# hasindu2008/sigfish

Hardware: AMD Instinct MI355X
Metric: reads/s (sDTW alignment stage: nCoV-2019 R9 DNA, -q 250, both strands) (higher is better)
Workload: dtype f32

## Files before the change

### sigfish_amd/csrc/sdtw_kernels.hpp

```cpp
#pragma once

#include <hip/hip_runtime.h>
#include <stddef.h>
#include <stdint.h>

#include "row_rules.hpp"

namespace sfa {

constexpr int kRefPad = 128;
#ifndef SFA_STEPS_PER_LOAD
#define SFA_STEPS_PER_LOAD 4
#endif
#ifndef SFA_FILL_WAVES
#define SFA_FILL_WAVES 6
#endif
#ifndef SFA_FILL32_WAVES
#define SFA_FILL32_WAVES 4
#endif
#ifndef SFA_LCK_WAVES
#define SFA_LCK_WAVES 4
#endif
#ifndef SFA_TRACE_WAVES
#define SFA_TRACE_WAVES 4
// ... 1169 lines not shown
template <int MAXR, bool STD, bool LCK = false>
__global__ void __launch_bounds__(256, MAXR <= 16 ? SFA_TRACE_WAVES : 1) sdtw_trace_kernel(const DpArgs a, int32_t *out_st) {
    const int task = __builtin_amdgcn_readfirstlane(blockIdx.x * 4 + (threadIdx.x >> 6));
    if (task >= a.n_tasks) return;
    int ci = 0;
    while (ci + 1 < a.n_cls && task >= a.cls[ci + 1].task_base) ++ci;
    const ClassDesc cd = a.cls[ci];
    const int tl = task - cd.task_base;
    __shared__ float lds_f[4 * kXchWordsPerWave];
    __shared__ int lds_i[4 * kXchWordsPerWave];
#define SFA_SHAPE(RR, LL)                                                                    \
    case (RR) * 256 + (LL):                                                                  \
        if constexpr (MAXR >= (RR)) trace_body<RR, LL, STD, LCK>(a, cd, tl, out_st, lds_f, lds_i); \
        break;
    switch (cd.R * 256 + cd.lanes) {
        SFA_SHAPE(32, 64) SFA_SHAPE(32, 32) SFA_SHAPE(32, 16)
        SFA_SHAPE(16, 64) SFA_SHAPE(16, 32) SFA_SHAPE(16, 16)
        SFA_SHAPE(8, 64) SFA_SHAPE(8, 32) SFA_SHAPE(8, 16)
        SFA_SHAPE(4, 64) SFA_SHAPE(4, 32)
        default:
            trace_body<4, 16, STD, LCK>(a, cd, tl, out_st, lds_f, lds_i);
            break;
    }
#undef SFA_SHAPE
}

template <int R, int L, bool STD, bool LCK>
__device__ __forceinline__ void fused_trace_task(const DpArgs &a, const ClassDesc cd, const int quad_local, float *lds_f, int *lds_i, float *lds_x) {
    const int quad = cd.quad_base + quad_local;
    const int lane = threadIdx.x & 63;
    const int g = lane & (L - 1);
    const int slot = lane / L;
    int seen;
    const bool arrived = bounded_wait_ge(a.quad_done + quad, a.n_chunks, a.spin_limit, &seen, true);
    __builtin_amdgcn_fence(__ATOMIC_ACQUIRE, "agent");
    __builtin_amdgcn_wave_barrier();
    if (!arrived) {
        if (lane == 0) report_device_error(a.err, kErrQuadWait, quad, seen);
        return;
    }
    const int qlen = __builtin_amdgcn_readfirstlane(a.quad_qlen[quad]);
    const int lq = (qlen - 1) / R;
    const int read = a.order[quad * 4 + slot];
    const bool owner = (g == lq) && read >= 0;
    ResultRow r = no_row();
    Winner w;
    w.job = -1;
    w.ws = -1;
    w.best = 0.0f;
    w.chunk = 0;
    if (owner && !a.bad[read]) {
        float best = INFINITY, second = INFINITY;
        int end = -1, job = -1, chunk = 0;
        for (int ch = 0; ch < a.n_chunks; ++ch) {
            const int64_t o = (static_cast<int64_t>(quad) * a.n_chunks + ch) * 4 + slot;
            const float b = a.p_best[o], s2 = a.p_second[o];
            const float hi = fmaxf(best, b);
            const float lo2 = fminf(second, s2);
            const bool take = !(b > best);
            second = fminf(hi, lo2);
            if (take) {
                best = b;
                end = a.p_end[o];
                job = a.p_job[o];
                chunk = ch;
            }
        }
        r.valid = 1;
        r.score = best;
        r.score2 = second;
        if (job >= 0) {
            r.rid = a.job_contig[job];
            r.strand = a.job_strand[job];
            r.mapq = mapq_from_scores(best, second);
            w.job = job;
            w.ws = end;
            w.best = best;
            w.chunk = chunk;
        }
    }
    const int src = (lane & ~(L - 1)) + lq;
    w.job = __shfl(w.job, src);
    w.ws = __shfl(w.ws, src);
    w.best = __shfl(w.best, src);
    w.chunk = __shfl(w.chunk, src);
    int res_st, res_end;
    trace_core<R, L, STD, LCK, (R == 32)>(a, cd, quad_local, w, lds_f, lds_i, res_st, res_end, lds_x);
    if (owner) {
        if (r.rid >= 0) {
            const int rl = a.ref_len[r.rid], off = a.ref_st_offset[r.rid];
            r.pos_st = ((r.strand == '+') ? res_st : rl - res_end) + off;
            r.pos_end = ((r.strand == '+') ? res_end : rl - res_st) + off;
            if (a.span_hist && res_st >= 0 && res_end >= res_st) {
                const int64_t ql = a.q_off[read + 1] - a.q_off[read];
                if (ql > 0) {
                    const int64_t b = (static_cast<int64_t>(res_end - res_st + 1) * 16) / ql;
                    atomicAdd(a.span_hist + (b < kSpanBuckets - 1 ? static_cast<int>(b) : kSpanBuckets - 1), 1u);
                }
            }
        }
        a.out[read] = r;
    }
}

template <int MAXR, bool STD, bool LCK>
__device__ __attribute__((noinline)) void fused_trace_dispatch(const DpArgs *pa, const int quad, float *lds_f, int *lds_i, float *lds_x) {
    const DpArgs &a = *pa;
    int ci = 0;
    while (ci + 1 < a.n_cls && quad >= a.cls[ci + 1].quad_base) ++ci;
    const ClassDesc cd = a.cls[ci];
    const int ql = quad - cd.quad_base;
#define SFA_TSHAPE(RR, LL)                                                               \
    case (RR) * 256 + (LL):                                                              \
        if constexpr (MAXR >= (RR)) fused_trace_task<RR, LL, STD, LCK>(a, cd, ql, lds_f, lds_i, lds_x); \
        break;
    switch (cd.R * 256 + cd.lanes) {
        SFA_TSHAPE(32, 64) SFA_TSHAPE(32, 32) SFA_TSHAPE(32, 16)
        SFA_TSHAPE(16, 64) SFA_TSHAPE(16, 32) SFA_TSHAPE(16, 16)
        SFA_TSHAPE(8, 64) SFA_TSHAPE(8, 32) SFA_TSHAPE(8, 16)
        SFA_TSHAPE(4, 64) SFA_TSHAPE(4, 32) SFA_TSHAPE(4, 16)
        default:
            break;
    }
#undef SFA_TSHAPE
}

struct SecArgs {
    const int32_t *slot_of_read;
    const int32_t *p_top5;
    const uint8_t *bad;
    const int64_t *q_off;
    int32_t max_query;
    int32_t n_reads, n_chunks;
    int32_t *s_job;
    int32_t *s_end;
// ... 29 lines not shown
    if (w >= static_cast<int64_t>(n_quads_total) * per_quad) return;
    const int quad = static_cast<int>(w / per_quad), rest = static_cast<int>(w - static_cast<int64_t>(quad) * per_quad);
    const int job = rest / (a.n_seg - 1), seg = rest - job * (a.n_seg - 1);
    int ci = 0;
    while (ci + 1 < a.n_cls && quad >= a.cls[ci + 1].quad_base) ++ci;
    const int qlen = a.quad_qlen[quad];
    const SegRange next = segment_range(a.job_len[job], qlen, a.n_seg, a.warm_windows, seg + 1);
    if (next.empty) return;
    const int lane = threadIdx.x & 63;
    const float *out = a.verify + verify_slot(a, quad, job, seg, 1) + lane, *in = a.verify + verify_slot(a, quad, job, seg + 1, 0) + lane;
    bool same = true;
    for (int p = 0; p <= a.cls[ci].R; ++p) same = same && (__float_as_uint(out[p * 64]) == __float_as_uint(in[p * 64]));
    if (!__all(same) && lane == 0) a.seg_fail[quad] = 1;
}

__global__ void __launch_bounds__(256) sdtw_screen_kernel(const float *queries, const int64_t *q_off, const int n, uint8_t *bad,
                                                          unsigned *count) {
    const int i = blockIdx.x * 4 + (threadIdx.x >> 6);
    if (i >= n) return;
    const int lane = threadIdx.x & 63;
    const int64_t b = q_off[i], e = q_off[i + 1];
    bool nf = false;
    for (int64_t j = b + lane; j < e; j += 64) {
        const unsigned u = __float_as_uint(queries[j]);
        nf = nf || ((u & 0x7f800000u) == 0x7f800000u);
    }
    const bool any = __any(nf);
    if (lane == 0) {
        bad[i] = any ? 1 : 0;
        if (any) atomicAdd(count, 1u);
    }
}

struct ChunkWin {
    int end, job, chunk;
};
__global__ void __launch_bounds__(256) sdtw_finalize_kernel(const FinalizeArgs a) {
    const int i = blockIdx.x * blockDim.x + threadIdx.x;
    if (i >= a.n_reads) return;
    const int sl = a.slot_of_read[i];
    const int64_t qlen = a.q_off[i + 1] - a.q_off[i];
    const bool strips = a.max_query > 0 && qlen > a.max_query;
    if (strips && a.mode != 1) return;
    if (a.mode == 3) {
        if (sl < 0) a.out[i] = no_row();
        return;
    }
    if (a.mode == 2) {
        if (sl < 0) return;
        ResultRow r = a.out[i];
        if (r.rid < 0) return;
        const int st = a.t_st[i];
        const int end = a.t_st[a.n_reads + i];
        place_row(r, st, end, a.ref);
        a.out[i] = r;
        const int b = a.span_hist ? span_bucket(st, end, qlen) : -1;
        if (b >= 0) atomicAdd(a.span_hist + b, 1u);
        return;
    }
    const bool on = sl >= 0 && !a.bad[i];
    Top2Merge<ChunkWin> m({-1, -1, 0});
    for (int ch = 0; on && ch < a.n_chunks; ++ch) {
        const int64_t o = (static_cast<int64_t>(sl >> 2) * a.n_chunks + ch) * 4 + (sl & 3);
        m.offer(a.p_best[o], a.p_second[o], {a.p_end[o], a.p_job[o], ch});
    }
    const ResultRow r = on ? primary_row(m.best, m.second, m.pay.job, a.ref) : no_row();
// ... 12 lines not shown
```

### sigfish_amd/csrc/sfa_align.hip

```cpp
#define SFA_DEFINE_FINALIZE_KERNEL
#include "sfa_ctx.hpp"
#include "sdtw_instances.hpp"
#include "sdtw_strips.hpp"

using sfa::DpArgs;
using sfa::FinalizeArgs;
using sfa::Route;
using sfa::SecArgs;
using sfa::ResultRow;
using sfa::align_device;
using sfa::for_each_shard;
using sfa::for_each_shard_range;
using sfa::resolve_profile;

namespace {

template <int Cap, typename F>
void by_rows(int maxr, F f) {
    if constexpr (Cap >= 32) {
        if (maxr >= 32) return f(std::integral_constant<int, 32>());
    }
    if (maxr >= 16) return f(std::integral_constant<int, 16>());
    if (maxr >= 8) return f(std::integral_constant<int, 8>());
    f(std::integral_constant<int, 4>());
// ... 227 lines not shown
        sum.n_tasks += c->prof.n_tasks;
        sum.n_chunks = std::max(sum.n_chunks, c->prof.n_chunks);
        sum.non_finite_reads += c->prof.non_finite_reads;
        sum.lck_fallbacks += c->prof.lck_fallbacks;
        sum.lck_from_scratch += c->prof.lck_from_scratch;
    }
    c->prof = sum;
    return SFA_OK;
}


bool fused(Route r) { return r == Route::LdsFused || r == Route::Fused32; }
bool lds(Route r) { return r == Route::Lds || r == Route::LdsFused; }

sfa::PlanParams plan_params(const sfa_ctx *c) {
    sfa::PlanParams pp;
    pp.n_sims = static_cast<int64_t>(c->cu_count) * 4;
    pp.waves_per_simd = c->opt_waves_per_simd;
    pp.ckpt_interval = c->opt_ckpt_interval;
    pp.ckpt_budget_bytes = c->opt_ckpt_budget;
    pp.trace_margin = c->opt_trace_margin;
    pp.lane_widening = c->opt_lane_widening;
    pp.widen_below = c->opt_widen_below;
    pp.column_segments = c->opt_column_segments;
    pp.segment_warm_windows = c->opt_segment_warm;
    pp.std_dtw = (c->flag & SFA_DTW) != 0;
    pp.span_sixteenths = c->wave.span_sixteenths;
    pp.allow_segments = !pp.std_dtw && !c->seg.no_segments_once && c->opt_secondary == 0;
    pp.lds_ckpt = c->opt_secondary > 0 ? 0 : static_cast<int>(c->opt_lds_ckpt);
    return pp;
}

struct Staging {
    size_t order, qq, slot, chunk, ckoff, bytes;
    Staging(int32_t n, const sfa::BatchPlan &p, int32_t n_jobs) {
        order = sizeof(int64_t) * (n + 1);
        qq = order + sizeof(int32_t) * 4 * std::max(p.n_quads, 1);
        slot = qq + sizeof(int32_t) * std::max(p.n_quads, 1);
        chunk = slot + sizeof(int32_t) * n;
        ckoff = chunk + sizeof(int32_t) * (p.n_chunks + 1);
        bytes = ckoff + sizeof(int32_t) * (n_jobs + 1);
    }
};

int stage_and_reserve(sfa_ctx *c, const int64_t *q_off, int32_t n, Route route, const Staging &sg) {
    const sfa::BatchPlan &plan = c->wave.plan;
    const int32_t n_quads = plan.n_quads, n_chunks = plan.n_chunks, n_jobs = c->model.n_jobs;
    const size_t n_part = static_cast<size_t>(std::max(n_quads, 1)) * n_chunks * 4, nr = static_cast<size_t>(n);
    int rc;
    if ((rc = c->wave.reserve(sg.bytes, n_part, nr, plan.ck_floats)) || (rc = c->status.reserve(nr))) return rc;
    if (c->opt_secondary > 0 && (rc = c->sec.reserve(n_part, nr))) return rc;
    if (fused(route) && (rc = c->fused.reserve(static_cast<size_t>(std::max(n_quads, 1))))) return rc;
    if (lds(route) && (rc = c->lds.reserve(n_part, nr))) return rc;
    if (route == Route::Segments && (rc = c->seg.reserve(plan, n_jobs))) return rc;
    char *hs = c->wave.h_stage.as<char>();
    memcpy(hs, q_off, sizeof(int64_t) * (n + 1));
    memcpy(hs + sg.order, plan.order.data(), sizeof(int32_t) * plan.order.size());
    memcpy(hs + sg.qq, plan.quad_qlen.data(), sizeof(int32_t) * plan.quad_qlen.size());
    memcpy(hs + sg.slot, plan.slot_of_read.data(), sizeof(int32_t) * n);
    memcpy(hs + sg.chunk, plan.chunk_begin.data(), sizeof(int32_t) * (n_chunks + 1));
    memcpy(hs + sg.ckoff, plan.job_ck_off.data(), sizeof(int32_t) * (n_jobs + 1));
#ifdef SFA_TASK_TIMES
    if ((rc = c->times.d_times.reserve(24 * static_cast<size_t>(std::max(n_quads * n_chunks, 1))))) return rc;
    c->times.n_times = n_quads * n_chunks;
#endif
    return SFA_OK;
}

struct BatchArgs {
    DpArgs da{};
    FinalizeArgs fz{};
    SecArgs sa{};
};

BatchArgs batch_args(sfa_ctx *c, const float *d_queries, int32_t n, ResultRow *d_out, ResultRow *d_sec, Route route, const Staging &sg,
                     bool has_long) {
    const sfa::BatchPlan &plan = c->wave.plan;
    const int32_t n_quads = plan.n_quads, n_chunks = plan.n_chunks, n_jobs = c->model.n_jobs;
    const char *ds = c->wave.d_stage.as<char>();
    BatchArgs a;
    DpArgs &da = a.da;
    da.queries = d_queries;
    da.q_off = reinterpret_cast<const int64_t *>(ds);
    da.order = reinterpret_cast<const int32_t *>(ds + sg.order);
    da.quad_qlen = reinterpret_cast<const int32_t *>(ds + sg.qq);
    da.ref = c->model.d_ref.as<float>();
    da.job_off = c->model.d_job_off.as<int64_t>();
    da.job_len = c->model.d_job_len.as<int32_t>();
    da.chunk_begin = reinterpret_cast<const int32_t *>(ds + sg.chunk);
    da.job_ck_off = reinterpret_cast<const int32_t *>(ds + sg.ckoff);
    da.ck = c->wave.d_ck.as<float>();
    da.p_best = c->wave.d_pbest.as<float>();
    da.p_end = c->wave.d_pend.as<int32_t>();
    da.p_job = c->wave.d_pjob.as<int32_t>();
    da.p_second = c->wave.d_psecond.as<float>();
    da.w_job = c->wave.d_wjob.as<int32_t>();
    da.w_end = c->wave.d_wend.as<int32_t>();
// ... 21 lines not shown
    da.seg_fail = c->seg.d_segfail.as<int32_t>();
    da.best_rec = c->lds.d_bestrec.as<float>();
    da.best_e = c->lds.d_beste.as<int32_t>();
    da.g_best = c->lds.d_gbest.as<unsigned>();
    da.w_chunk = c->wave.d_wchunk.as<int32_t>();
    da.best_planes = sfa::kLdsCkPlanes;
    da.ticket = c->fused.d_ticket.as<unsigned>();
    da.quad_done = c->fused.d_quaddone.as<int32_t>();
    da.n_quads_total = n_quads;
    const sfa::RefTables ref = c->model.tables();
    da.job_contig = ref.job_contig;
    da.job_strand = ref.job_strand;
    da.ref_len = ref.ref_len;
    da.ref_st_offset = ref.ref_st_offset;
    da.bad = c->status.d_bad.as<uint8_t>();
    da.out = d_out;
    da.span_hist = route == Route::Fused32 ? c->status.dev()->span_hist : nullptr;
    da.prio_unit = static_cast<int32_t>(c->opt_prio_unit);
    da.started = c->wave.d_started.as<unsigned>();
    da.err = c->status.dev()->err;
    da.lck_stats = &c->status.dev()->lck_fallbacks;
    {
        int64_t longest = 0;
        for (int32_t ch = 0; ch < n_chunks; ++ch) {
            int64_t cols = 0;
            for (int32_t j = plan.chunk_begin[ch]; j < plan.chunk_begin[ch + 1] && j < n_jobs; ++j) cols += c->model.h_job_len[j];
            longest = std::max(longest, cols);
        }
        da.spin_limit = std::max<int64_t>(c->opt_spin_limit_ms, longest / 1000) * 100000;
        c->wave.quad_limit_ms = da.spin_limit / 100000;
    }
    da.debug_drop_quad = static_cast<int32_t>(c->opt_debug_drop_quad);
    da.p_top5 = route == Route::Secondary ? c->sec.d_p5.as<int32_t>() : nullptr;
    da.self = fused(route) ? c->fused.d_args.as<DpArgs>() : nullptr;
#ifdef SFA_TASK_TIMES
    da.task_times = c->times.d_times.as<unsigned long long>();
#endif

    FinalizeArgs &fz = a.fz;
    fz.slot_of_read = reinterpret_cast<const int32_t *>(ds + sg.slot);
    fz.p_best = da.p_best;
    fz.p_end = da.p_end;
    fz.p_job = da.p_job;
    fz.p_second = da.p_second;
    fz.ref = ref;
    fz.w_job = da.w_job;
    fz.w_end = da.w_end;
    fz.w_score = da.w_score;
    fz.w_chunk = da.w_chunk;
    fz.t_st = c->wave.d_tst.as<int32_t>();
    fz.out = d_out;
    fz.bad = da.bad;
    fz.q_off = da.q_off;
    fz.max_query = has_long ? sfa::kMaxQuery : 0;
    fz.n_reads = n;
    fz.n_chunks = n_chunks;
    fz.span_hist = c->status.dev()->span_hist;

    if (c->opt_secondary > 0) {
        SecArgs &sa = a.sa;
        sa.slot_of_read = fz.slot_of_read;
        sa.p_top5 = c->sec.d_p5.as<int32_t>();
        sa.bad = fz.bad;
        sa.q_off = fz.q_off;
        sa.max_query = fz.max_query;
        sa.n_reads = n;
        sa.n_chunks = n_chunks;
        sa.s_job = c->sec.d_swin.as<int32_t>();
        sa.s_end = sa.s_job + 5 * static_cast<size_t>(n);
        sa.s_score = reinterpret_cast<float *>(sa.s_end + 5 * static_cast<size_t>(n));
        sa.t_st = c->sec.d_sts.as<int32_t>();
        sa.ref = ref;
        sa.sec = d_sec;
        sa.n_sec = static_cast<int32_t>(c->opt_secondary);
    }
    return a;
}

int launch_finalize(FinalizeArgs fz, int mode, hipStream_t st) {
    fz.mode = mode;
    hipLaunchKernelGGL(sfa::sdtw_finalize_kernel, dim3((fz.n_reads + 255) / 256), dim3(256), 0, st, fz);
    KERNEL_TRY();
    return SFA_OK;
}

int enqueue_pass1(sfa_ctx *c, Route route, const BatchArgs &a, hipStream_t st) {
    if (route == Route::NoQuads) return SFA_OK;
    const DpArgs &da = a.da;
    const int32_t n_quads = da.n_quads_total;
    if (lds(route))
        HIP_TRY(hipMemsetD32Async(reinterpret_cast<hipDeviceptr_t>(c->lds.d_gbest.p), 0x7f800000, static_cast<size_t>(da.n_reads_total), st));
    if (fused(route)) {
        HIP_TRY(hipMemsetAsync(c->fused.d_ticket.p, 0, 4, st));
        HIP_TRY(hipMemsetAsync(c->fused.d_quaddone.p, 0, 4 * static_cast<size_t>(n_quads), st));
        if (int rc = launch_finalize(a.fz, 3, st)) return rc;
        HIP_TRY(hipMemcpyAsync(c->fused.d_args.p, &da, sizeof(DpArgs), hipMemcpyHostToDevice, st));
    }
    const int maxr = c->wave.plan.max_R;
    const dim3 block(256), grid((da.n_tasks + 3) / 4), fgrid(static_cast<unsigned>((da.n_tasks + 3) / 4 + (n_quads + 3) / 4));
    by_std((c->flag & SFA_DTW) != 0, [&](auto S) {
        if (route == Route::Segments)
            by_rows<32>(maxr, [&](auto R) { hipLaunchKernelGGL((sfa::sdtw_fill_kernel<R, false, true>), grid, block, 0, st, da); });
        else if (route == Route::Lds)
            by_rows<16>(maxr, [&](auto R) { hipLaunchKernelGGL((sfa::sdtw_fill_kernel<R, S, false, true>), grid, block, 0, st, da); });
        else if (route == Route::LdsFused)
            by_rows<16>(maxr, [&](auto R) { hipLaunchKernelGGL((sfa::sdtw_fill_kernel<R, S, false, true, true>), fgrid, block, 0, st, da); });
        else if (route == Route::Fused32)
            hipLaunchKernelGGL((sfa::sdtw_fill_kernel<32, false, false, false, true>), fgrid, block, 0, st, da);
        else if (route == Route::Secondary)
            by_rows<32>(maxr, [&](auto R) { hipLaunchKernelGGL((sfa::sdtw_sec_fill_kernel<R, S>), grid, block, 0, st, da); });
        else
            by_rows<32>(maxr, [&](auto R) { hipLaunchKernelGGL((sfa::sdtw_fill_kernel<R, S>), grid, block, 0, st, da); });
    });
    KERNEL_TRY();
    if (route == Route::Segments) {
        HIP_TRY(hipMemsetAsync(c->seg.d_segfail.p, 0, 4 * static_cast<size_t>(n_quads), st));
        const int64_t waves = static_cast<int64_t>(n_quads) * da.n_jobs * (da.n_seg - 1);
        hipLaunchKernelGGL(sfa::sdtw_verify_kernel, dim3(static_cast<unsigned>((waves + 3) / 4)), dim3(256), 0, st, da, n_quads);
        KERNEL_TRY();
    }
    return SFA_OK;
}

void launch_pass2(sfa_ctx *c, Route route, DpArgs ta, int32_t *out_st, hipStream_t st) {
    for (int i = 0; i < ta.n_cls; ++i) ta.cls[i].task_base = ta.cls[i].quad_base;
// ... 18 lines not shown
    }
    HIP_TRY(hipEventRecord(c->ev[3], st));
    return own_launch ? launch_finalize(a.fz, 2, st) : SFA_OK;
}

int enqueue_secondaries(sfa_ctx *c, Route route, const BatchArgs &a, hipStream_t st) {
    SecArgs sa = a.sa;
    const int32_t n = sa.n_reads;
    const dim3 fgrid((n + 255) / 256), fblock(256);
    sa.mode = 1;
    hipLaunchKernelGGL(sfa::sdtw_sec_finalize_kernel, fgrid, fblock, 0, st, sa);
    KERNEL_TRY();
    for (int k = 1; k <= sa.n_sec && route == Route::Secondary; ++k) {
        DpArgs ta = a.da;
        ta.w_job = sa.s_job + static_cast<size_t>(k) * n;
        ta.w_end = sa.s_end + static_cast<size_t>(k) * n;
        ta.w_score = sa.s_score + static_cast<size_t>(k) * n;
        launch_pass2(c, route, ta, c->sec.d_sts.as<int32_t>() + 2 * static_cast<size_t>(k) * n, st);
        KERNEL_TRY();
    }
    sa.mode = 2;
    hipLaunchKernelGGL(sfa::sdtw_sec_finalize_kernel, fgrid, fblock, 0, st, sa);
    KERNEL_TRY();
    return SFA_OK;
}

int enqueue_batch(sfa_ctx *c, Route route, const BatchArgs &a, const sfa::LongPlan &lp) {
    hipStream_t st = c->stream;
    const DpArgs &da = a.da;
    int rc;
    if (da.prio_unit > 0) HIP_TRY(hipMemsetAsync(c->wave.d_started.p, 0, 4, st));
    HIP_TRY(hipEventRecord(c->ev[0], st));
    HIP_TRY(hipMemsetAsync(c->status.dev(), 0, sizeof(sfa::BatchStatus), st));
    hipLaunchKernelGGL(sfa::sdtw_screen_kernel, dim3((da.n_reads_total + 3) / 4), dim3(256), 0, st, da.queries, da.q_off, da.n_reads_total, c->status.d_bad.as<uint8_t>(),
                       &c->status.dev()->non_finite);
    KERNEL_TRY();
    if (!lp.reads.empty()) {
        hipStream_t ls = c->stream_long;
        HIP_TRY(hipEventRecord(c->lev[0], st));
        HIP_TRY(hipStreamWaitEvent(ls, c->lev[0], 0));
        if ((rc = align_long(c, lp, da.queries, da.q_off, da.out, a.sa.sec, ls))) {
            (void)hipStreamSynchronize(ls);
            (void)hipStreamSynchronize(c->stream_long2);
            return rc;
        }
        HIP_TRY(hipEventRecord(c->lev[1], ls));
    }
    if ((rc = enqueue_pass1(c, route, a, st))) return rc;
    HIP_TRY(hipEventRecord(c->ev[1], st));
    if ((rc = enqueue_pass2(c, route, a, st))) return rc;
    if (c->opt_secondary > 0 && (rc = enqueue_secondaries(c, route, a, st))) return rc;
    c->prof.fill_launches = (route != Route::NoQuads ? 1 : 0) + lp.n_groups;
    c->strips.long_pending = !lp.reads.empty();
    if (c->strips.long_pending) {
        HIP_TRY(hipEventRecord(c->ev[5], st));
        HIP_TRY(hipStreamWaitEvent(st, c->lev[1], 0));
        if (strip_secondaries(c) && a.sa.sec) {
            sfa::StripSecArgs xa = strip_sec_args(c, lp, 0, lp.n_long(), a.sa.sec);
            xa.mode = 2;
            hipLaunchKernelGGL(sfa::sdtw_strip_sec_finalize_kernel, dim3((xa.n_long + 63) / 64), dim3(64), 0, st, xa);
            KERNEL_TRY();
        }
    }
    HIP_TRY(hipMemcpyAsync(c->status.h_block.p, c->status.dev(), sizeof(sfa::BatchStatus), hipMemcpyDeviceToHost, st));
    HIP_TRY(hipEventRecord(c->ev[4], st));

    const sfa::BatchPlan &plan = c->wave.plan;
    c->prof.cells = (plan.query_events + lp.events) * c->model.total_cols;
// ... 15 lines not shown
int sfa::align_device(sfa_ctx *c, const float *d_queries, const int64_t *q_off, int32_t n, ResultRow *d_out, ResultRow *d_sec) {
    if (!c->in_slice && !c->seg.no_segments_once) {
        c->maps.map_n = n;
        c->maps.map_q_off.assign(q_off, q_off + n + 1);
        c->maps.map_queries = d_queries;
    }
    if (n == 0) return SFA_OK;
    const int n_sec = static_cast<int>(c->opt_secondary);
    const bool own_sec = n_sec > 0 && !d_sec;
    if (own_sec) {
        c->sec.sec_n = -1;
        if (int rc = c->sec.reserve_rows(static_cast<size_t>(n))) return rc;
        d_sec = c->sec.d_sec.as<ResultRow>();
    }
    const sfa::LongPlan lp = sfa::plan_long_reads(q_off, n, c->model.h_job_len, c->opt_ckpt_interval, c->opt_ckpt_budget, c->cu_count, c->opt_spin_limit_ms);
    sfa::PlanParams pp = plan_params(c);
    pp.skip_long = !lp.reads.empty();
    sfa::BatchPlan &plan = c->wave.plan;
    std::string perr;
    if (int rc = sfa::plan_batch(q_off, n, c->model.h_job_len, c->model.total_cols, pp, &plan, &perr)) return fail(rc, "%s", perr.c_str());
    if (!c->in_slice && c->opt_ckpt_interval == 0 && plan.ck_shift > 9 && n >= 2 * c->opt_min_slice_reads) {
        const int64_t want = (plan.ck_floats * 4 * (1ll << (plan.ck_shift - 9)) + pp.ckpt_budget_bytes - 1) / std::max<int64_t>(pp.ckpt_budget_bytes, 1);
        const int32_t slices = static_cast<int32_t>(std::min<int64_t>(want, n / c->opt_min_slice_reads));
        if (slices > 1) {
            const int rc = align_sliced(c, d_queries, q_off, n, d_out, d_sec, slices);
            if (!rc && own_sec) c->sec.sec_n = n;
            return rc;
        }
    }
    const Route route = sfa::choose_route(plan, pp.std_dtw, n_sec, c->opt_fused_trace, static_cast<int64_t>(c->cu_count) * 4 * SFA_LCK_WAVES);
    const Staging sg(n, plan, c->model.n_jobs);
    int rc;
    if ((rc = stage_and_reserve(c, q_off, n, route, sg))) return rc;
    HIP_TRY(hipMemcpyAsync(c->wave.d_stage.p, c->wave.h_stage.p, sg.bytes, hipMemcpyHostToDevice, c->stream));
    const BatchArgs a = batch_args(c, d_queries, n, d_out, d_sec, route, sg, !lp.reads.empty());
    if ((rc = enqueue_batch(c, route, a, lp))) return rc;
    if (route == Route::Segments) {
        int32_t *flags = c->seg.h_flags.as<int32_t>();
        HIP_TRY(hipMemcpyAsync(flags, c->seg.d_segfail.p, 4 * static_cast<size_t>(plan.n_quads), hipMemcpyDeviceToHost, c->stream));
        HIP_TRY(hipStreamSynchronize(c->stream));
        if (std::any_of(flags, flags + plan.n_quads, [](int32_t f) { return f != 0; })) {
            c->seg.no_segments_once = true;
            rc = align_device(c, d_queries, q_off, n, d_out);
            c->seg.no_segments_once = false;
            c->seg.seg_reruns++;
            c->prof.segment_reruns = c->seg.seg_reruns;
            return rc;
        }
    }
    if (own_sec) c->sec.sec_n = n;
    return SFA_OK;
}

int sfa::resolve_profile(sfa_ctx *c) {
    if (!c->prof_pending) return SFA_OK;
    HIP_TRY(hipEventSynchronize(c->ev[4]));
    float a = 0, b = 0, d = 0, t = 0;
    HIP_TRY(hipEventElapsedTime(&a, c->ev[0], c->ev[1]));
    HIP_TRY(hipEventElapsedTime(&b, c->ev[1], c->ev[2]));
    HIP_TRY(hipEventElapsedTime(&d, c->ev[2], c->ev[3]));
    HIP_TRY(hipEventElapsedTime(&t, c->ev[0], c->ev[4]));
    if (c->prof.fused_trace) d = 0;
    if (c->strips.long_pending) {
        float l = 0;
        HIP_TRY(hipEventElapsedTime(&l, c->ev[5], c->ev[4]));
        a += l;
        a = t;
        d = 0;
// ... 206 lines not shown
```

### sigfish_amd/csrc/sfa_context.hip

```cpp
#include "sfa_ctx.hpp"

namespace sfa {
std::string &last_error_slot() {
    thread_local std::string err;
    return err;
}
}
using sfa::resolve_profile;

extern "C" {

const char *sfa_last_error(void) { return sfa::last_error_slot().c_str(); }
void sfa_set_error_(const char *msg) { sfa::last_error_slot() = msg ? msg : ""; }
const char *sfa_version(void) { return SFA_VERSION; }
#ifndef SFA_BUILD_ID
#define SFA_BUILD_ID "unknown"
#endif
const char *sfa_build_id(void) { return SFA_BUILD_ID; }

}

struct HostRef {
    int32_t num_ref = 0, n_jobs = 0;
    int64_t total_cols = 0;
// ... 157 lines not shown
        return SFA_OK;
    }
    const std::string k(key);
    if (k == "ckpt_interval") {
        if (value != 0 && (value < 4 || (value & (value - 1)))) return fail(SFA_EINVAL, "ckpt_interval must be 0 or a power of two >= 4");
        c->opt_ckpt_interval = value;
    } else if (k == "ckpt_budget_bytes") {
        if (value < 0) return fail(SFA_EINVAL, "ckpt_budget_bytes must be >= 0");
        c->opt_ckpt_budget = value;
    } else if (k == "trace_margin") {
        if (value < -1 || value > (1 << 28)) return fail(SFA_EINVAL, "trace_margin must be -1 (auto) .. 2^28");
        c->opt_trace_margin = value;
    } else if (k == "lane_widening") {
        if (value != 0 && value != 1 && value != 2 && value != 4) return fail(SFA_EINVAL, "lane_widening must be 0 (auto), 1, 2 or 4");
        c->opt_lane_widening = value;
    } else if (k == "widen_below") {
        if (value < 0 || value > 64) return fail(SFA_EINVAL, "widen_below must be 0..64");
        c->opt_widen_below = value;
    } else if (k == "column_segments") {
        if (value < 0 || value > 64) return fail(SFA_EINVAL, "column_segments must be 0 (auto), 1 (off) or 2..64");
        c->opt_column_segments = value;
    } else if (k == "segment_warm_windows") {
        if (value < 0 || value > 64) return fail(SFA_EINVAL, "segment_warm_windows must be 0..64");
        c->opt_segment_warm = value;
    } else if (k == "min_slice_reads") {
        if (value < 1) return fail(SFA_EINVAL, "min_slice_reads must be >= 1");
        c->opt_min_slice_reads = value;
    } else if (k == "waves_per_simd") {
        if (value < 1 || value > 8) return fail(SFA_EINVAL, "waves_per_simd must be 1..8");
        c->opt_waves_per_simd = value;
    } else if (k == "fused_trace") {
        if (value < 0 || value > 2) return fail(SFA_EINVAL, "fused_trace must be 0 (off), 1 (launches with more tasks than wave slots) or 2 (always)");
        c->opt_fused_trace = value;
    } else if (k == "lds_ckpt") {
        if (value < 0 || value > 2) return fail(SFA_EINVAL, "lds_ckpt must be 0 (off), 1 (where shapes and batch size suit) or 2 (wherever the shapes allow)");
        c->opt_lds_ckpt = value;
    } else if (k == "secondary") {
        if (value < 0 || value > 4) return fail(SFA_EINVAL, "secondary must be 0..4 (secondary mappings per read)");
        c->opt_secondary = value;
    } else if (k == "secondary_strips") {
        if (value != 0 && value != 1) return fail(SFA_EINVAL, "secondary_strips must be 0 (reads beyond SFA_MAX_QUERY events have no secondaries) or 1 (the row strips keep their lists)");
        c->opt_secondary_strips = value;
    } else if (k == "map_scratch_bytes") {
        if (value < 0) return fail(SFA_EINVAL, "map_scratch_bytes must be >= 0");
        c->opt_map_scratch = value;
    } else if (k == "map_strips") {
        if (value != 0 && value != 1) return fail(SFA_EINVAL, "map_strips must be 0 (rows beyond SFA_MAX_QUERY events on the host) or 1 (on the device, in row strips)");
        c->opt_map_strips = value;
    } else if (k == "prio_unit") {
        if (value < 0 || value > (1 << 28)) return fail(SFA_EINVAL, "prio_unit must be 0 (off) .. 2^28");
        c->opt_prio_unit = value;
    } else if (k == "spin_limit_ms") {
        if (value < 1 || value > 3600000) return fail(SFA_EINVAL, "spin_limit_ms must be 1 .. 3 600 000");
        c->opt_spin_limit_ms = value;
    } else if (k == "ev_parallel") {
        if (value < 0 || value > 3) return fail(SFA_EINVAL, "ev_parallel must be 0..3 (bit 0: prefix sums, bit 1: peak picker)");
        c->opt_ev_parallel = value;
    } else if (k == "zstd_tables") {
        if (value != 0 && value != 1) return fail(SFA_EINVAL, "zstd_tables must be 0 (the device zstd decoder keeps its tables in HBM scratch) or 1 (in LDS)");
        c->opt_zstd_tables = value;
    } else if (k == "debug_drop_quad" || k == "debug_drop_strip") {
        const char *e = getenv("SFA_TEST_HOOKS");
        if (!e || strcmp(e, "1") != 0) return fail(SFA_EINVAL, "'%s' is a test hook: set SFA_TEST_HOOKS=1 in the environment to use it", key);
        if (value < -1 || value > INT32_MAX) return fail(SFA_EINVAL, "%s must be -1 (off) or an index", key);
        (k == "debug_drop_quad" ? c->opt_debug_drop_quad : c->opt_debug_drop_strip) = value;
    } else {
// ... 102 lines not shown
```

### sigfish_amd/csrc/sfa_ctx.hpp

```cpp
#pragma once
#include <hip/hip_runtime.h>

#include <algorithm>
#include <cmath>
#include <condition_variable>
#include <cstdarg>
#include <cstdio>
#include <cstdlib>
#include <cstring>
#include <functional>
#include <memory>
#include <mutex>
#include <string>
#include <thread>
#include <vector>

#include "../../include/sigfish_amd.h"
#include "sdtw_kernels.hpp"
#include "sfa_buf.hpp"
#include "sfa_plan.hpp"

namespace {

int fail(int code, const char *fmt, ...) {
// ... 292 lines not shown
};

}

struct sfa_ctx {
    std::vector<sfa_ctx *> shards;
    std::vector<std::unique_ptr<ShardWorker>> workers;
    std::vector<int32_t> shard_lo;

    int device = 0;
    uint32_t flag = 0;
    int pore = 0;
    int cu_count = 256;
    Stream stream;
    Stream stream_long;
    Stream stream_long2;
    Event lev[4];
    Event eev[4];
    Event ev[6];
    Event bev[2];

    int64_t opt_ckpt_interval = 0;
    int64_t opt_ckpt_budget = 32ll << 30;
    int64_t opt_ev_parallel = 3;
    int64_t opt_zstd_tables = 1;
    int64_t opt_min_slice_reads = 65536;
    int64_t opt_segment_warm = 4;
    int64_t opt_column_segments = 0;
    int64_t opt_lane_widening = 0;
    int64_t opt_widen_below = 5;
    int64_t opt_trace_margin = -1;
    int64_t opt_waves_per_simd = 6;
    int64_t opt_fused_trace = 1;
    int64_t opt_lds_ckpt = 1;
    int64_t opt_secondary = 0;
    int64_t opt_secondary_strips = 0;
    int64_t opt_prio_unit = 2048;
    int64_t opt_spin_limit_ms = 20000;
    int64_t opt_debug_drop_quad = -1;
    int64_t opt_debug_drop_strip = -1;
    int64_t opt_map_scratch = 2ll << 30;
    int64_t opt_map_strips = 0;

    ctx::RefModel model;
    ctx::CallerIO io;
    ctx::Status status;
    ctx::WaveKernels wave;
    ctx::FusedLaunch fused;
    ctx::LdsRoute lds;
    ctx::Segments seg;
    ctx::Strips strips;
    ctx::Secondaries sec;
    ctx::RawSignal raw;
    ctx::Blow5 blow5;
    ctx::EventMaps maps;
    ctx::TaskTimes times;
    sfa_profile_t prof{};
    bool prof_pending = false;
    bool in_slice = false;
    std::vector<struct sfa_session *> sessions;
};

namespace sfa {
void destroy_sessions(sfa_ctx *c);
int resolve_profile(sfa_ctx *c);
int align_device(sfa_ctx *c, const float *d_queries, const int64_t *q_off, int32_t n, struct ResultRow *d_out,
// ... 37 lines not shown
```

### sigfish_amd/csrc/sfa_plan.hpp

```cpp
#pragma once

#include <algorithm>
#include <cstdint>
#include <string>
#include <vector>

namespace sfa {

constexpr int kMaxQuery = 2048;

struct ClassShape {
    int R, lanes;
};
constexpr ClassShape kClassShapes[6] = {{32, 64}, {32, 32}, {32, 16}, {16, 16}, {8, 16}, {4, 16}};

inline ClassShape widened(int ci, int w) {
    ClassShape s = kClassShapes[ci];
    while (w > 1 && s.lanes < 64 && s.R > 4) {
        s.R /= 2;
        s.lanes *= 2;
        w /= 2;
    }
    return s;
}
// ... 41 lines not shown
    std::vector<int32_t> job_ck_off;
    std::vector<PlanClass> classes;
    std::vector<int32_t> s_qlen, s_count, s_fill_pos, s_slot_start, s_len_quad_base;
    std::vector<int8_t> s_per_shift;
    void reset() {
        n_quads = 0; n_chunks = 1; max_R = 4; max_lanes = 16; widening = 1; ck_shift = 0; trace_margin = 0;
        n_seg = 1; warm_windows = 4;
        lds_ckpt = false;
        ck_floats = 0; query_events = 0;
        classes.clear();
    }
};

inline void split_jobs(const std::vector<int32_t> &job_len, int64_t total_cols, int32_t n_chunks, int32_t *chunk_begin) {
    const int32_t n_jobs = static_cast<int32_t>(job_len.size());
    int64_t acc = 0;
    int32_t j = 0;
    chunk_begin[0] = 0;
    for (int32_t ch = 1; ch < n_chunks; ++ch) {
        const int64_t want = total_cols * ch / n_chunks;
        acc += job_len[j++];
        while (j < n_jobs - (n_chunks - ch) && acc + job_len[j] / 2 < want) acc += job_len[j++];
        chunk_begin[ch] = j;
    }
    chunk_begin[n_chunks] = n_jobs;
}

inline int plan_batch(const int64_t *q_off, int32_t n, const std::vector<int32_t> &job_len, int64_t total_cols,
                      const PlanParams &pp, BatchPlan *out, std::string *err) {
    BatchPlan &p = *out;
    p.reset();
    const int32_t n_jobs = static_cast<int32_t>(job_len.size());
    std::vector<int32_t> &qlen = p.s_qlen, &count = p.s_count, &fill_pos = p.s_fill_pos;
    qlen.assign(n, 0);
    count.assign(kMaxQuery + 2, 0);
    int maxq = 0;
    for (int32_t i = 0; i < n; ++i) {
        const int64_t l = q_off[i + 1] - q_off[i];
        if (l < 0) {
            *err = "q_off is not monotone at read " + std::to_string(i);
            return -1;
        }
        if (l > kMaxQuery && pp.skip_long) continue;
        if (l > kMaxQuery) {
            *err = "read " + std::to_string(i) + " has " + std::to_string(l) + " events; the limit is " + std::to_string(kMaxQuery);
            return -4;
        }
        qlen[i] = static_cast<int32_t>(l);
        count[l]++;
        maxq = std::max(maxq, qlen[i]);
        p.query_events += l;
    }
    auto mixing = [&](int w) { return !pp.std_dtw && w < 4; };
    std::vector<int32_t> &slot_start = p.s_slot_start, &len_quad_base = p.s_len_quad_base;
    slot_start.assign(maxq + 2, 0);
    len_quad_base.assign(maxq + 2, 0);
    auto layout = [&](int w) {
        p.classes.clear();
        int32_t n_quads = 0;
        const bool mix = mixing(w);
        for (int ci = 0; ci < 6; ++ci) {
            const ClassShape sh = widened(ci, w);
            PlanClass cl;
            cl.R = sh.R;
            cl.lanes = sh.lanes;
            cl.quad_base = n_quads;
            const int per = 64 / cl.lanes;
            int32_t pos = 0;
            const int n_res = mix ? cl.R : 1;
            for (int res = 0; res < n_res; ++res) {
                for (int l = maxq; l >= 1; --l) {
                    if (count[l] == 0 || class_for(l) != ci || (mix && l % cl.R != res)) continue;
                    slot_start[l] = pos;
                    len_quad_base[l] = cl.quad_base;
                    pos += count[l];
                    if (!mix) pos = (pos + per - 1) / per * per;
                }
                pos = (pos + per - 1) / per * per;
            }
            n_quads += pos / per;
            cl.n_quads = n_quads - cl.quad_base;
            if (cl.n_quads > 0) p.classes.push_back(cl);
        }
        return n_quads;
    };
    auto chunks_for = [&](int32_t n_quads) -> int32_t {
        if (n_quads <= 0 || n_jobs <= 1) return 1;
        const int64_t target = pp.n_sims * pp.waves_per_simd * 16;
        return static_cast<int32_t>(std::min<int64_t>(n_jobs, std::max<int64_t>(1, (target + n_quads - 1) / n_quads)));
    };
    int w = 1;
    int32_t n_quads = layout(1);
    if (pp.lane_widening > 0) {
        w = static_cast<int>(pp.lane_widening);
        if (w != 1) n_quads = layout(w);
    } else {
        const int64_t tasks1 = static_cast<int64_t>(n_quads) * chunks_for(n_quads);
        if (tasks1 * 5 < pp.widen_below * pp.n_sims * 4) {
            w = (tasks1 * 50 < pp.widen_below * pp.n_sims * 9) ? 4 : 2;
            n_quads = layout(w);
        }
    }
    p.widening = w;
    p.n_quads = n_quads;
    p.max_R = 4;
    p.max_lanes = 16;
    for (const PlanClass &cl : p.classes) {
        p.max_R = std::max(p.max_R, cl.R);
        p.max_lanes = std::max(p.max_lanes, cl.lanes);
    }
    p.order.assign(4 * static_cast<size_t>(std::max(n_quads, 1)), -1);
    p.quad_qlen.assign(std::max(n_quads, 1), 0);
    p.slot_of_read.assign(n, -1);
    fill_pos.assign(maxq + 2, 0);
    std::vector<int8_t> &per_shift = p.s_per_shift;
    per_shift.assign(maxq + 2, 0);
    for (int l = 1; l <= maxq; ++l)
        if (count[l]) {
            const int per = 64 / widened(class_for(l), w).lanes;
            per_shift[l] = per == 4 ? 2 : (per == 2 ? 1 : 0);
        }
    for (int32_t i = 0; i < n; ++i) {
        const int l = qlen[i];
        if (l == 0) continue;
        const int32_t k = slot_start[l] + fill_pos[l]++;
        const int sh = per_shift[l];
        const int32_t qd = len_quad_base[l] + (k >> sh);
        const int32_t sl = qd * 4 + (k & ((1 << sh) - 1));
        p.order[sl] = i;
        p.slot_of_read[i] = sl;
        p.quad_qlen[qd] = std::max(p.quad_qlen[qd], l);
    }
    if (n_quads == 0) p.quad_qlen[0] = 1;

    if (pp.allow_segments && p.widening == 4 && p.max_lanes == 64 && n_quads > 0) {
        int32_t min_len = n_jobs ? job_len[0] : 0;
        for (int32_t j = 1; j < n_jobs; ++j) min_len = std::min(min_len, job_len[j]);
        const int64_t tasks = static_cast<int64_t>(n_quads) * n_jobs;
        int64_t S = pp.column_segments > 0 ? pp.column_segments : ((pp.widen_below + 1) * pp.n_sims + tasks - 1) / tasks;
        S = std::min<int64_t>(S, 64);
        S = std::min<int64_t>(S, min_len / (4 * std::max<int64_t>(pp.segment_warm_windows, 1) * std::max(maxq, 1)));
        if (S >= 3 || (pp.column_segments > 1 && S >= 2)) p.n_seg = static_cast<int32_t>(S);
        p.warm_windows = static_cast<int32_t>(pp.segment_warm_windows);
    }
    if (p.n_seg > 1) {
        p.n_chunks = n_jobs * p.n_seg;
        p.chunk_begin.resize(p.n_chunks + 1);
        for (int32_t c = 0; c < p.n_chunks; ++c) p.chunk_begin[c] = c / p.n_seg;
        p.chunk_begin[p.n_chunks] = n_jobs;
    } else {
        p.n_chunks = chunks_for(n_quads);
        p.chunk_begin.resize(p.n_chunks + 1);
        split_jobs(job_len, total_cols, p.n_chunks, p.chunk_begin.data());
    }

    p.job_ck_off.assign(n_jobs + 1, 0);
    p.trace_margin = static_cast<int32_t>(pp.trace_margin >= 0 ? pp.trace_margin : maxq + p.max_lanes);
    const bool adapt = pp.trace_margin < 0 && pp.span_sixteenths > 0;
    p.lds_ckpt = pp.lds_ckpt && pp.ckpt_interval == 0 && p.max_R <= 16 && p.n_seg == 1 && n_quads > 0 && maxq <= (pp.lds_ckpt >= 2 ? 1024 : 256);
    {
        const int64_t tasks = static_cast<int64_t>(n_quads) * p.n_chunks;
        if (pp.lds_ckpt < 2 && tasks > 4 * pp.n_sims && tasks <= 6 * pp.n_sims) p.lds_ckpt = false;
    }
    if (p.lds_ckpt && !pp.std_dtw) p.trace_margin = std::min<int32_t>(p.trace_margin, maxq - (maxq - 1) / p.max_R);
// ... 240 lines not shown
```

Before: 1.359 million.

## Fuse pre-launch memsets into one prepare kernel and streamline host planning

Adds an optional sdtw_prepare_kernel that folds the ticket, quad_done and g_best resets, the no-row finalize pass and the non-finite screen into one launch. The DpArgs are also staged in the same host-to-device copy instead of a separate buffer. The host planner loops are rewritten to batch length-run counting and cache per-length slot state, which cuts per-read work. The fused prepare path is off by default (opt_fused_prepare = 0), so with default settings only the planner change and task-timing instrumentation apply.

```diff
diff --git a/sigfish_amd/csrc/sdtw_kernels.hpp b/sigfish_amd/csrc/sdtw_kernels.hpp
--- a/sigfish_amd/csrc/sdtw_kernels.hpp
+++ b/sigfish_amd/csrc/sdtw_kernels.hpp
@@ -1225,9 +1225,16 @@
     const int g = lane & (L - 1);
     const int slot = lane / L;
     int seen;
+#ifdef SFA_TASK_TIMES
+    unsigned long long *const dbg_times = a.task_times ? a.task_times + 3 * (static_cast<int64_t>(a.n_tasks) + quad) : nullptr;
+    if (dbg_times && lane == 0) dbg_times[0] = wall_clock64();
+#endif
     const bool arrived = bounded_wait_ge(a.quad_done + quad, a.n_chunks, a.spin_limit, &seen, true);
     __builtin_amdgcn_fence(__ATOMIC_ACQUIRE, "agent");
     __builtin_amdgcn_wave_barrier();
+#ifdef SFA_TASK_TIMES
+    if (dbg_times && lane == 0) dbg_times[2] = wall_clock64();
+#endif
     if (!arrived) {
         if (lane == 0) report_device_error(a.err, kErrQuadWait, quad, seen);
         return;
@@ -1294,6 +1301,9 @@
         }
         a.out[read] = r;
     }
+#ifdef SFA_TASK_TIMES
+    if (dbg_times && lane == 0) dbg_times[1] = wall_clock64();
+#endif
 }
 
 template <int MAXR, bool STD, bool LCK>
@@ -1389,6 +1399,45 @@
     }
 }
 
+struct PrepareArgs {
+    const float *queries;
+    const int64_t *q_off;
+    int32_t n_reads, n_quads;
+    uint8_t *bad;
+    unsigned *non_finite;
+    unsigned *g_best;
+    unsigned *ticket;
+    int32_t *quad_done;
+    const int32_t *slot_of_read;
+    ResultRow *out;
+    int32_t max_query;
+};
+__global__ void __launch_bounds__(256) sdtw_prepare_kernel(const PrepareArgs a) {
+    const int64_t gid = static_cast<int64_t>(blockIdx.x) * 256 + threadIdx.x;
+    if (gid == 0) *a.ticket = 0;
+    if (gid < a.n_quads) a.quad_done[gid] = 0;
+    if (gid < a.n_reads) {
+        if (a.g_best) a.g_best[gid] = 0x7f800000u;
+        const int64_t qlen = a.q_off[gid + 1] - a.q_off[gid];
+        const bool strips = a.max_query > 0 && qlen > a.max_query;
+        if (!strips && a.slot_of_read[gid] < 0) a.out[gid] = no_row();
+    }
+    const int i = blockIdx.x * 4 + (threadIdx.x >> 6);
+    if (i >= a.n_reads) return;
+    const int lane = threadIdx.x & 63;
+    const int64_t b = a.q_off[i], e = a.q_off[i + 1];
+    bool nf = false;
+    for (int64_t j = b + lane; j < e; j += 64) {
+        const unsigned u = __float_as_uint(a.queries[j]);
+        nf = nf || ((u & 0x7f800000u) == 0x7f800000u);
+    }
+    const bool any = __any(nf);
+    if (lane == 0) {
+        a.bad[i] = any ? 1 : 0;
+        if (any) atomicAdd(a.non_finite, 1u);
+    }
+}
+
 struct ChunkWin {
     int end, job, chunk;
 };
diff --git a/sigfish_amd/csrc/sfa_align.hip b/sigfish_amd/csrc/sfa_align.hip
--- a/sigfish_amd/csrc/sfa_align.hip
+++ b/sigfish_amd/csrc/sfa_align.hip
@@ -283,14 +283,15 @@
 }
 
 struct Staging {
-    size_t order, qq, slot, chunk, ckoff, bytes;
+    size_t order, qq, slot, chunk, ckoff, args, bytes;
     Staging(int32_t n, const sfa::BatchPlan &p, int32_t n_jobs) {
         order = sizeof(int64_t) * (n + 1);
         qq = order + sizeof(int32_t) * 4 * std::max(p.n_quads, 1);
         slot = qq + sizeof(int32_t) * std::max(p.n_quads, 1);
         chunk = slot + sizeof(int32_t) * n;
         ckoff = chunk + sizeof(int32_t) * (p.n_chunks + 1);
-        bytes = ckoff + sizeof(int32_t) * (n_jobs + 1);
+        args = (ckoff + sizeof(int32_t) * (n_jobs + 1) + 15) & ~static_cast<size_t>(15);
+        bytes = args + sizeof(DpArgs);
     }
 };
 
@@ -312,8 +313,8 @@
     memcpy(hs + sg.chunk, plan.chunk_begin.data(), sizeof(int32_t) * (n_chunks + 1));
     memcpy(hs + sg.ckoff, plan.job_ck_off.data(), sizeof(int32_t) * (n_jobs + 1));
 #ifdef SFA_TASK_TIMES
-    if ((rc = c->times.d_times.reserve(24 * static_cast<size_t>(std::max(n_quads * n_chunks, 1))))) return rc;
-    c->times.n_times = n_quads * n_chunks;
+    c->times.n_times = static_cast<int64_t>(n_quads) * n_chunks + (fused(route) ? n_quads : 0);
+    if ((rc = c->times.d_times.reserve(24 * static_cast<size_t>(std::max<int64_t>(c->times.n_times, 1))))) return rc;
 #endif
     return SFA_OK;
 }
@@ -401,7 +402,7 @@
     }
     da.debug_drop_quad = static_cast<int32_t>(c->opt_debug_drop_quad);
     da.p_top5 = route == Route::Secondary ? c->sec.d_p5.as<int32_t>() : nullptr;
-    da.self = fused(route) ? c->fused.d_args.as<DpArgs>() : nullptr;
+    da.self = !fused(route) ? nullptr : (c->opt_fused_prepare ? reinterpret_cast<const DpArgs *>(ds + sg.args) : c->fused.d_args.as<DpArgs>());
 #ifdef SFA_TASK_TIMES
     da.task_times = c->times.d_times.as<unsigned long long>();
 #endif
@@ -457,9 +458,10 @@
     if (route == Route::NoQuads) return SFA_OK;
     const DpArgs &da = a.da;
     const int32_t n_quads = da.n_quads_total;
-    if (lds(route))
+    const bool prepared = fused(route) && c->opt_fused_prepare;
+    if (lds(route) && !prepared)
         HIP_TRY(hipMemsetD32Async(reinterpret_cast<hipDeviceptr_t>(c->lds.d_gbest.p), 0x7f800000, static_cast<size_t>(da.n_reads_total), st));
-    if (fused(route)) {
+    if (fused(route) && !prepared) {
         HIP_TRY(hipMemsetAsync(c->fused.d_ticket.p, 0, 4, st));
         HIP_TRY(hipMemsetAsync(c->fused.d_quaddone.p, 0, 4 * static_cast<size_t>(n_quads), st));
         if (int rc = launch_finalize(a.fz, 3, st)) return rc;
@@ -544,8 +546,25 @@
     if (da.prio_unit > 0) HIP_TRY(hipMemsetAsync(c->wave.d_started.p, 0, 4, st));
     HIP_TRY(hipEventRecord(c->ev[0], st));
     HIP_TRY(hipMemsetAsync(c->status.dev(), 0, sizeof(sfa::BatchStatus), st));
-    hipLaunchKernelGGL(sfa::sdtw_screen_kernel, dim3((da.n_reads_total + 3) / 4), dim3(256), 0, st, da.queries, da.q_off, da.n_reads_total, c->status.d_bad.as<uint8_t>(),
-                       &c->status.dev()->non_finite);
+    if (fused(route) && c->opt_fused_prepare) {
+        sfa::PrepareArgs pa{};
+        pa.queries = da.queries;
+        pa.q_off = da.q_off;
+        pa.n_reads = da.n_reads_total;
+        pa.n_quads = da.n_quads_total;
+        pa.bad = c->status.d_bad.as<uint8_t>();
+        pa.non_finite = &c->status.dev()->non_finite;
+        pa.g_best = lds(route) ? da.g_best : nullptr;
+        pa.ticket = da.ticket;
+        pa.quad_done = da.quad_done;
+        pa.slot_of_read = a.fz.slot_of_read;
+        pa.out = da.out;
+        pa.max_query = a.fz.max_query;
+        hipLaunchKernelGGL(sfa::sdtw_prepare_kernel, dim3((da.n_reads_total + 3) / 4), dim3(256), 0, st, pa);
+    } else {
+        hipLaunchKernelGGL(sfa::sdtw_screen_kernel, dim3((da.n_reads_total + 3) / 4), dim3(256), 0, st, da.queries, da.q_off, da.n_reads_total, c->status.d_bad.as<uint8_t>(),
+                           &c->status.dev()->non_finite);
+    }
     KERNEL_TRY();
     if (!lp.reads.empty()) {
         hipStream_t ls = c->stream_long;
@@ -627,8 +646,9 @@
     const Staging sg(n, plan, c->model.n_jobs);
     int rc;
     if ((rc = stage_and_reserve(c, q_off, n, route, sg))) return rc;
+    const BatchArgs a = batch_args(c, d_queries, n, d_out, d_sec, route, sg, !lp.reads.empty());
+    if (fused(route) && c->opt_fused_prepare) memcpy(c->wave.h_stage.as<char>() + sg.args, &a.da, sizeof(DpArgs));
     HIP_TRY(hipMemcpyAsync(c->wave.d_stage.p, c->wave.h_stage.p, sg.bytes, hipMemcpyHostToDevice, c->stream));
-    const BatchArgs a = batch_args(c, d_queries, n, d_out, d_sec, route, sg, !lp.reads.empty());
     if ((rc = enqueue_batch(c, route, a, lp))) return rc;
     if (route == Route::Segments) {
         int32_t *flags = c->seg.h_flags.as<int32_t>();
diff --git a/sigfish_amd/csrc/sfa_context.hip b/sigfish_amd/csrc/sfa_context.hip
--- a/sigfish_amd/csrc/sfa_context.hip
+++ b/sigfish_amd/csrc/sfa_context.hip
@@ -213,6 +213,9 @@
     } else if (k == "fused_trace") {
         if (value < 0 || value > 2) return fail(SFA_EINVAL, "fused_trace must be 0 (off), 1 (launches with more tasks than wave slots) or 2 (always)");
         c->opt_fused_trace = value;
+    } else if (k == "fused_prepare") {
+        if (value != 0 && value != 1) return fail(SFA_EINVAL, "fused_prepare must be 0 (memsets and kernels of their own in front of a fused launch) or 1 (one kernel)");
+        c->opt_fused_prepare = value;
     } else if (k == "lds_ckpt") {
         if (value < 0 || value > 2) return fail(SFA_EINVAL, "lds_ckpt must be 0 (off), 1 (where shapes and batch size suit) or 2 (wherever the shapes allow)");
         c->opt_lds_ckpt = value;
diff --git a/sigfish_amd/csrc/sfa_ctx.hpp b/sigfish_amd/csrc/sfa_ctx.hpp
--- a/sigfish_amd/csrc/sfa_ctx.hpp
+++ b/sigfish_amd/csrc/sfa_ctx.hpp
@@ -348,6 +348,7 @@
     int64_t opt_trace_margin = -1;
     int64_t opt_waves_per_simd = 6;
     int64_t opt_fused_trace = 1;
+    int64_t opt_fused_prepare = 0;
     int64_t opt_lds_ckpt = 1;
     int64_t opt_secondary = 0;
     int64_t opt_secondary_strips = 0;
diff --git a/sigfish_amd/csrc/sfa_plan.hpp b/sigfish_amd/csrc/sfa_plan.hpp
--- a/sigfish_amd/csrc/sfa_plan.hpp
+++ b/sigfish_amd/csrc/sfa_plan.hpp
@@ -97,25 +97,37 @@
     p.reset();
     const int32_t n_jobs = static_cast<int32_t>(job_len.size());
     std::vector<int32_t> &qlen = p.s_qlen, &count = p.s_count, &fill_pos = p.s_fill_pos;
-    qlen.assign(n, 0);
+    qlen.resize(n);
     count.assign(kMaxQuery + 2, 0);
     int maxq = 0;
+    int32_t run_l = 0, run_n = 0;
+    int64_t events = 0;
     for (int32_t i = 0; i < n; ++i) {
         const int64_t l = q_off[i + 1] - q_off[i];
         if (l < 0) {
             *err = "q_off is not monotone at read " + std::to_string(i);
             return -1;
         }
-        if (l > kMaxQuery && pp.skip_long) continue;
+        if (l > kMaxQuery && pp.skip_long) {
+            qlen[i] = 0;
+            continue;
+        }
         if (l > kMaxQuery) {
             *err = "read " + std::to_string(i) + " has " + std::to_string(l) + " events; the limit is " + std::to_string(kMaxQuery);
             return -4;
         }
         qlen[i] = static_cast<int32_t>(l);
-        count[l]++;
+        if (qlen[i] != run_l) {
+            count[run_l] += run_n;
+            run_l = qlen[i];
+            run_n = 0;
+        }
+        ++run_n;
         maxq = std::max(maxq, qlen[i]);
-        p.query_events += l;
-    }
+        events += l;
+    }
+    count[run_l] += run_n;
+    p.query_events = events;
     auto mixing = [&](int w) { return !pp.std_dtw && w < 4; };
     std::vector<int32_t> &slot_start = p.s_slot_start, &len_quad_base = p.s_len_quad_base;
     slot_start.assign(maxq + 2, 0);
@@ -176,7 +188,7 @@
     }
     p.order.assign(4 * static_cast<size_t>(std::max(n_quads, 1)), -1);
     p.quad_qlen.assign(std::max(n_quads, 1), 0);
-    p.slot_of_read.assign(n, -1);
+    p.slot_of_read.resize(n);
     fill_pos.assign(maxq + 2, 0);
     std::vector<int8_t> &per_shift = p.s_per_shift;
     per_shift.assign(maxq + 2, 0);
@@ -185,16 +197,31 @@
             const int per = 64 / widened(class_for(l), w).lanes;
             per_shift[l] = per == 4 ? 2 : (per == 2 ? 1 : 0);
         }
-    for (int32_t i = 0; i < n; ++i) {
-        const int l = qlen[i];
-        if (l == 0) continue;
-        const int32_t k = slot_start[l] + fill_pos[l]++;
-        const int sh = per_shift[l];
-        const int32_t qd = len_quad_base[l] + (k >> sh);
-        const int32_t sl = qd * 4 + (k & ((1 << sh) - 1));
-        p.order[sl] = i;
-        p.slot_of_read[i] = sl;
-        p.quad_qlen[qd] = std::max(p.quad_qlen[qd], l);
+    {
+        int32_t *const order = p.order.data(), *const slot_of_read = p.slot_of_read.data(), *const quad_qlen = p.quad_qlen.data();
+        int cur = 0, sh = 0;
+        int32_t k = 0, quad_base = 0;
+        for (int32_t i = 0; i < n; ++i) {
+            const int l = qlen[i];
+            if (l == 0) {
+                slot_of_read[i] = -1;
+                continue;
+            }
+            if (l != cur) {
+                if (cur) fill_pos[cur] = k - slot_start[cur];
+                cur = l;
+                k = slot_start[l] + fill_pos[l];
+                sh = per_shift[l];
+                quad_base = len_quad_base[l];
+            }
+            const int32_t qd = quad_base + (k >> sh);
+            const int32_t sl = qd * 4 + (k & ((1 << sh) - 1));
+            ++k;
+            order[sl] = i;
+            slot_of_read[i] = sl;
+            if (quad_qlen[qd] < l) quad_qlen[qd] = l;
+        }
+        if (cur) fill_pos[cur] = k - slot_start[cur];
     }
     if (n_quads == 0) p.quad_qlen[0] = 1;
 
```

Result: no change. 1.359 million (-0.0%).
